# HybridRobotics/ilqr-iterative-tasks

Hardware: AMD Instinct MI355X
Metric: batched iLQR iterations/s (n=6,m=2,N=20) (higher is better)
Workload: dtype f64

## Files before the change

ilqr_iterative_tasks_amd/csrc/i2lqr_abi.hip:

```cpp
#include <hip/hip_runtime.h>

#include <atomic>
#include <cmath>
#include <cstdarg>
#include <cstdio>
#include <cstdlib>
#include <cstring>
#include <mutex>
#include <new>
#include <unordered_set>

#include "../../include/i2lqr.h"
#include "i2lqr_devcfg.hpp"
#include "i2lqr_geometry.hpp"
#include "i2lqr_group.h"
#include "i2lqr_handle.hpp"
#include "i2lqr_host.hpp"
#include "i2lqr_kernels.h"
#include "i2lqr_lane12.h"
#include "i2lqr_rccl.hpp"
#include "i2lqr_select.hpp"
#include "i2lqr_wave_opt.h"

#include "i2lqr_lane_launch.hpp"
// ... 491 lines not shown
  if (!h->lane_models) return refuse_layout(what);
  if (h->cfg.system_id == I2LQR_SYS_QUAD12)
    return fail(I2LQR_ERR_UNSUPPORTED, "%s with \"lane_models\" is built for the bicycles' "
                "one-problem-per-lane kernel, not for quad12's row-block kernel "
                "(k_lane_iterate_rows): use the problem-major layout", what);
  return I2LQR_OK;
}

int i2lqr_set_option(i2lqr_handle* h, const char* name, int64_t value) {
  if (!h || !name) return fail(I2LQR_ERR_INVALID, "null handle or option name");
  if (value < -1 || value > 0x7fffffff) return fail(I2LQR_ERR_INVALID, "option value out of range");
  const int v = (int)value;
  LaneTune& lane = h->lane;
  ColumnTune& col = h->col;
  if (!strcmp(name, "defer_states")) lane.opt_defer = v < 0 ? -1 : (v != 0);
  else if (!strcmp(name, "reroll_nominal")) lane.opt_reroll = v < 0 ? -1 : (v != 0);
  else if (!strcmp(name, "lds_gain_steps")) lane.opt_lds_steps = v;
  else if (!strcmp(name, "merge_inputs")) lane.opt_merge = v < 0 ? -1 : (v != 0);
  else if (!strcmp(name, "checkpoint_states")) lane.opt_ckpt = v < 0 ? -1 : (v != 0);
  else if (!strcmp(name, "stagger")) lane.opt_stagger = v;
  else if (!strcmp(name, "per_step_jacobians")) col.opt_fstep = v < 0 ? -1 : (v != 0);
  else if (!strcmp(name, "wave_tail")) lane.wave_tail = v < 0 ? -1 : (v > 65536 ? 65536 : v);
  else if (!strcmp(name, "first_chunk")) lane.opt_first_chunk = v < 1 ? -1 : (v > 1024 ? 1024 : v);
  else if (!strcmp(name, "helper_wavefront")) lane.opt_pair = v < 0 ? -1 : (v != 0);
  else if (!strcmp(name, "state_buffers")) lane.opt_two_x = v < 0 ? -1 : (v != 0);
  else if (!strcmp(name, "chunk_step")) lane.opt_chunk_step = v < 1 ? -1 : (v > 1024 ? 1024 : v);
  else if (!strcmp(name, "fused_compaction")) lane.opt_fuse = v < 0 ? -1 : (v != 0);
  else if (!strcmp(name, "final_round")) lane.opt_final_round = v < 0 ? -1 : (v > 20 ? 20 : v);
  else if (!strcmp(name, "speculate")) col.opt_spec = v < 0 ? -1 : (v != 0);
  else if (!strcmp(name, "group_workspace")) col.opt_group_ws = v < 0 ? -1 : (v != 0);
  else if (!strcmp(name, "group_overlap")) col.opt_group_overlap = v < 0 ? -1 : (v != 0);
  else if (!strcmp(name, "group_fixed_horizon")) col.opt_group_fixed = v < 0 ? -1 : (v != 0);
  else if (!strcmp(name, "group_chains")) col.opt_group_chains = v < 0 ? -1 : (v != 0);
  else if (!strcmp(name, "debug_self_test")) {
#ifdef I2LQR_DEBUG
    unsigned long long* w = i2lqr::debug_trap_word();
    double* buf = nullptr;
    HIP_TRY(hipMalloc((void**)&buf, 8 * sizeof(double)));
    hipLaunchKernelGGL(k_debug_self_test, dim3(1), dim3(64), 0, (hipStream_t)0, buf, w);
    const int rc = debug_check(I2LQR_OK, nullptr);
    (void)hipFree(buf);
    return rc;
#else
    return fail(I2LQR_ERR_UNSUPPORTED, "\"debug_self_test\" exists in the index-checked debug build "
                "only (make -C ilqr_iterative_tasks_amd/csrc debug)");
#endif
  }
  else if (!strcmp(name, "line_search")) {
    if (v != -1 && v != 0 && v != 1 && v != 2 && v != 4 && v != 8)
      return fail(I2LQR_ERR_INVALID, "\"line_search\" is 2, 4 or 8 step sizes, or -1 / 0 / 1 (off)");
    if (v > 1 && !problem_major(h)) return refuse_layout(wave_phrase(WAVE_LS));
    h->model.ls = v > 1 ? v : 0;
  }
  else if (!strcmp(name, "obstacles")) {
    if (v > I2LQR_MAX_OBSTACLES)
      return fail(I2LQR_ERR_INVALID, "\"obstacles\" is 2 ... %d records per problem, or -1 / 0 / 1 "
                  "(off: one record)", I2LQR_MAX_OBSTACLES);
    if (v > 1)
      if (int rc = refuse_lane_model(h, wave_phrase(WAVE_OBS))) return rc;
    h->model.obs = v > 1 ? v : 0;
  }
  else if (!strcmp(name, "lane_models")) {
    if (v != -1 && v != 0 && v != 1)
      return fail(I2LQR_ERR_INVALID, "\"lane_models\" is 1 (on), or -1 / 0 (off)");
    if (v == 1 && problem_major(h))
      return fail(I2LQR_ERR_UNSUPPORTED, "\"lane_models\" is built for the batch-minor / batch-tiled "
// ... 611 lines not shown
```

ilqr_iterative_tasks_amd/csrc/i2lqr_column_launch.hpp:

```cpp
#pragma once
#include <hip/hip_runtime.h>

#include "i2lqr_column_plan.hpp"
#include "i2lqr_devcfg.hpp"
#include "i2lqr_group.h"
#include "i2lqr_handle.hpp"
#include "i2lqr_host.hpp"
#include "i2lqr_kernels.h"
#include "i2lqr_wave_opt.h"

namespace i2lqr {

inline thread_local i2lqr_handle::Epilogue* t_epi = nullptr;

inline int64_t registered_ws(const i2lqr_handle* h) { return h->ws ? h->ws_bytes : -1; }
inline ColumnChoice column_kernel(const i2lqr_handle* h, int64_t B, bool early_exit) {
  return column_kernel(h->geo, h->fit, h->col, h->model.form(), registered_ws(h), B, early_exit);
}

inline int wave_lds_check(const i2lqr_handle* h, bool chained) {
  const size_t need = wave_lds_need(h->fit, h->model, chained);
  if (need <= h->geo.max_dyn_lds) return I2LQR_OK;
  const WaveForm f = h->model.form(chained);
  const int n_obs = h->model.records();
// ... 6 lines not shown
  return fail(I2LQR_ERR_UNSUPPORTED, "horizon %d with %s needs %zu B of LDS per wavefront (> %zu KiB)",
              h->cfg.N, with, need, h->geo.max_dyn_lds / 1024);
}

template <class T, class Sys> struct Launch {
  static constexpr int n = Sys::n, m = Sys::m, LANES = 64;
  static constexpr bool kBicycle = m == 2 && n + m <= 8;
  using Cfg = DevCfg<T, n, m>;

  static unsigned grid(int64_t B) { return (unsigned)B; }

  static int prepare(i2lqr_handle* h) {
    h->lanes = LANES;
    h->fit.lds_wave = (size_t)Layout<Sys>(h->cfg.N).total * sizeof(T);
    h->fit.lds_wave_fstep = kWaveHasFstep<Sys> ? wave_fstep_lds_bytes<T, Sys>(h->cfg.N) : 0;
    const size_t lds = h->fit.lds_wave;
    if (lds > h->geo.max_dyn_lds)
      return fail(I2LQR_ERR_UNSUPPORTED, "horizon %d needs %zu B of LDS per wavefront (> %zu KiB)",
                  h->cfg.N, lds, h->geo.max_dyn_lds / 1024);
    if (lds > h->geo.default_dyn_lds)
      for (const void* kernel :
           {(const void*)k_iterate<T, Sys, LANES, false>, (const void*)k_iterate<T, Sys, LANES, true>,
            (const void*)k_backward<T, Sys, LANES, false>, (const void*)k_backward<T, Sys, LANES, true>,
            (const void*)k_forward<T, Sys, LANES, false>, (const void*)k_forward<T, Sys, LANES, true>,
            (const void*)k_rollout<T, Sys, LANES, false>, (const void*)k_rollout<T, Sys, LANES, true>})
        HIP_TRY(hipFuncSetAttribute(kernel, hipFuncAttributeMaxDynamicSharedMemorySize, (int)lds));
    return I2LQR_OK;
  }

  static int iterate(i2lqr_handle* h, const SolveIO& io, hipStream_t s) {
    const int64_t B = io.B;
    IterArgs<T> a = iter_args<T>(io);
    a.chains = h->col.opt_group_chains != 0;
#ifdef I2LQR_STAMPS
    a.dbg = (unsigned long long*)h->ws;
#endif
    const ColumnChoice choice = column_kernel(h, B, io.early_exit != 0);
    const ColumnKernel fk = choice.kernel;
    if (t_epi && (fk == K_GROUP || fk == K_GROUP16 || fk == K_GROUP_WS)) {
      a.qfun = t_epi->qfun;
      a.outer_iter = t_epi->outer_iter;
      a.max_relax_iter = t_epi->max_relax_iter;
      a.cost_it = (T*)t_epi->cost_it;
      if (t_epi->best_idx) {
        a.pick_part = (MinPair<T>*)t_epi->part;
        a.pick_ticket = h->ticket + h->ticket_next.fetch_add(1, std::memory_order_relaxed) %
                                        i2lqr_handle::kTickets;
        a.best_idx = t_epi->best_idx;
        a.best_cost = (T*)t_epi->best_cost;
      }
      t_epi->fused = true;
    }
#ifdef I2LQR_STAMPS
    constexpr bool stamps = true;
#else
    constexpr bool stamps = false;
#endif
    switch (fk) {
      case K_INVALID:
        return fail(I2LQR_ERR_UNSUPPORTED, "%s", choice.why);
      case K_SPEC:
      case K_SPEC16:
        if constexpr (kBicycle) {
          const int lanes = fk == K_SPEC16 ? 16 : 8;
          HIP_TRY(group_spec_iterate<T>(h->cfg, a, s, lanes,
                                        spec_wavefronts(h->geo, h->fit, lanes, B, false)));
// ... 106 lines not shown
```

ilqr_iterative_tasks_amd/csrc/i2lqr_column_plan.hpp:

```cpp
#pragma once
#include <cstddef>
#include <cstdint>
#include <cstdio>

#include "../../include/i2lqr.h"
#include "i2lqr_geometry.hpp"
#include "i2lqr_wave_model.hpp"

namespace i2lqr {

struct ColumnTune {
  int opt_fstep = -1;
  int opt_group = -1;
  int opt_spec = -1;
  int opt_group_ws = -1;
  int opt_group_overlap = -1;
  int opt_group_fixed = -1;
  int opt_group_chains = -1;
  int opt_wave_chain = 0;
};

struct ColumnFit {
  enum Plant { OTHER, BICYCLE, SIXTEEN };
  int plant = OTHER;
  bool weights = false;
  bool problem_major = false;
  bool f64 = true;
  int n = 0, N = 0, word = 8;
  bool fixed_horizon = false;
  size_t lds_wave = 0, lds_wave_fstep = 0;
  size_t lds_group8 = 0, lds_group16 = 0;
  size_t lds_group_ws = 0;
  size_t lds_spec8x2 = 0, lds_spec8x3 = 0;
  size_t lds_spec16x2 = 0, lds_spec16x3 = 0;
  size_t lds_quad = 0;
  int64_t ws_group = 0, ws_quad = 0;
};

constexpr int kEightLaneProblems = 8, kSixteenLaneProblems = 4;

constexpr int64_t kAutoGroupBatch = 1024;
constexpr int64_t kAutoSpecBatch = 12288;
constexpr int64_t kGroup16Batch = 4096;
constexpr int64_t kGroupWsBatch = 4096;
constexpr int64_t kGroupWsTop = 8192;
constexpr int64_t kGroupWsTopF32 = 7168;
constexpr int kSpecWideBatch = 512;

inline bool lds_fits(const DeviceGeometry& g, size_t bytes) { return bytes <= g.max_dyn_lds; }
inline bool column_plant_ok(const ColumnFit& f) { return f.plant == ColumnFit::BICYCLE && !f.weights; }
inline bool group_fits(const DeviceGeometry& g, const ColumnFit& f, int lanes) {
// ... 230 lines not shown
```

ilqr_iterative_tasks_amd/csrc/i2lqr_dryrun.hpp:

```cpp
#pragma once
#ifdef I2LQR_DRY_RUN
#include <hip/hip_runtime.h>

#include <cstddef>
#include <cstdint>

#include "i2lqr_wave.hpp"

namespace i2lqr {
namespace dry {

bool on();
void allow(const void* base, size_t bytes);
void reset();
void record(const char* expr, const void* kernel, dim3 grid, dim3 block, size_t lds);
void ptr(const char* field, const void* p);
void val(const char* field, int64_t v);
void end();
int64_t report(char* buf, int64_t n);

template <class A> inline void arg(const A&) {}
inline void arg(int64_t v) { val("int", v); }
inline void arg(int v) { val("int", v); }
template <class P> inline void arg(P* p) { ptr("pointer argument", (const void*)p); }
template <class T> inline void arg(const IterArgs<T>& a) {
  val("IterArgs.B", a.B); val("IterArgs.n_iters", a.n_iters); val("IterArgs.early_exit", a.early_exit);
  ptr("IterArgs.X", a.X); ptr("IterArgs.U", a.U); ptr("IterArgs.x_term", a.x_term);
  ptr("IterArgs.lamb", a.lamb); ptr("IterArgs.obs", a.obs); ptr("IterArgs.cost", a.cost);
  ptr("IterArgs.K", a.K); ptr("IterArgs.k", a.k); ptr("IterArgs.iters", a.iters);
  ptr("IterArgs.status", a.status); ptr("IterArgs.dbg", a.dbg); ptr("IterArgs.count", a.count);
  val("IterArgs.count_max", a.count_max); val("IterArgs.max_total", a.max_total);
  val("IterArgs.set_stride", a.set_stride);
  ptr("IterArgs.orig", a.orig); ptr("IterArgs.out_X", a.out_X);
  ptr("IterArgs.out_U", a.out_U); ptr("IterArgs.out_K", a.out_K);
  ptr("IterArgs.out_k", a.out_k); ptr("IterArgs.out_lamb", a.out_lamb);
  ptr("IterArgs.out_cost", a.out_cost); ptr("IterArgs.out_iters", a.out_iters);
  ptr("IterArgs.out_status", a.out_status);
  val("IterArgs.out_B", a.out_B); val("IterArgs.out_tiled", a.out_tiled);
  ptr("IterArgs.qfun", a.qfun);
  val("IterArgs.outer_iter", a.outer_iter); val("IterArgs.max_relax_iter", a.max_relax_iter);
  ptr("IterArgs.cost_it", a.cost_it); ptr("IterArgs.pick_part", a.pick_part);
  ptr("IterArgs.pick_ticket", a.pick_ticket); ptr("IterArgs.best_idx", a.best_idx);
  ptr("IterArgs.best_cost", a.best_cost); val("IterArgs.chain_len", a.chain_len);
  val("IterArgs.chains", a.chains);
}
#ifdef I2LQR_DRY_RUN_LANE
template <class T> inline void arg(const LaneSet<T>& s) {
  ptr("LaneSet.X", s.X); ptr("LaneSet.U", s.U); ptr("LaneSet.x_term", s.x_term);
  ptr("LaneSet.obs", s.obs); ptr("LaneSet.lamb", s.lamb); ptr("LaneSet.cost", s.cost);
  ptr("LaneSet.K", s.K); ptr("LaneSet.k", s.k); ptr("LaneSet.iters", s.iters);
  ptr("LaneSet.status", s.status); ptr("LaneSet.orig", s.orig); val("LaneSet.B", s.B);
}
template <class T> inline void arg(const LaneArgs<T>& a) {
  val("LaneArgs.B", a.B); val("LaneArgs.n_iters", a.n_iters); val("LaneArgs.early_exit", a.early_exit);
  ptr("LaneArgs.X", a.X); ptr("LaneArgs.U", a.U); ptr("LaneArgs.x_term", a.x_term);
  ptr("LaneArgs.lamb", a.lamb); ptr("LaneArgs.obs", a.obs); ptr("LaneArgs.cost", a.cost);
  ptr("LaneArgs.K", a.K); ptr("LaneArgs.k", a.k); ptr("LaneArgs.iters", a.iters);
  ptr("LaneArgs.status", a.status); ptr("LaneArgs.wsU", a.wsU); ptr("LaneArgs.wsK", a.wsK);
  ptr("LaneArgs.wsk", a.wsk); ptr("LaneArgs.wsX", a.wsX); ptr("LaneArgs.count", a.count);
  val("LaneArgs.resume", a.resume); val("LaneArgs.max_total", a.max_total);
  val("LaneArgs.count_lo", a.count_lo); val("LaneArgs.count_hi", a.count_hi);
  val("LaneArgs.two_max", a.two_max); val("LaneArgs.lds_grow", a.lds_grow);
  ptr("LaneArgs.dbg", a.dbg); val("LaneArgs.defer", a.defer);
  val("LaneArgs.lds_steps", a.lds_steps); val("LaneArgs.reroll", a.reroll);
  val("LaneArgs.merge", a.merge); val("LaneArgs.ckpt", a.ckpt); val("LaneArgs.stagger", a.stagger);
  val("LaneArgs.cp.on", a.cp.on);
  if (a.cp.on) {
    val("LaneArgs.cp.src_is_user", a.cp.src_is_user); val("LaneArgs.cp.user_tiled", a.cp.user_tiled);
    ptr("LaneArgs.cp.orig", a.cp.orig); ptr("LaneArgs.cp.count_out", a.cp.count_out);
    arg(a.cp.dst);
    arg(a.cp.usr);
  }
}
#endif

template <class... A>
inline void launch(const char* expr, const void* kernel, dim3 grid, dim3 block, size_t lds,
// ... 30 lines not shown
```

ilqr_iterative_tasks_amd/csrc/i2lqr_group.h:

```cpp
#pragma once
#include <hip/hip_runtime.h>

#include "../../include/i2lqr.h"
#include "i2lqr_column_plan.hpp"
#include "i2lqr_devcfg.hpp"
#include "i2lqr_wave.hpp"

namespace i2lqr {

inline ColumnFit column_fit_config(const i2lqr_config& cfg) {
  ColumnFit f;
  f.plant = cfg.m == 2 && cfg.n + cfg.m <= 8 ? ColumnFit::BICYCLE
            : cfg.n + cfg.m == 16 ? ColumnFit::SIXTEEN : ColumnFit::OTHER;
  f.weights = has_stage_weights(cfg);
  f.problem_major = cfg.layout == I2LQR_LAYOUT_PROBLEM_MAJOR;
  f.f64 = cfg.dtype == I2LQR_F64;
  f.n = cfg.n;
  f.N = cfg.N;
  f.word = f.f64 ? 8 : 4;
  return f;
}
void column_fit_group(const i2lqr_config& cfg, ColumnFit& fit);
void column_fit_quad(const i2lqr_config& cfg, ColumnFit& fit);

template <class T> hipError_t group_iterate(const i2lqr_config& cfg, const IterArgs<T>& a,
                                            hipStream_t stream, int wavefronts);

template <class T> hipError_t group16_iterate(const i2lqr_config& cfg, const IterArgs<T>& a,
                                              hipStream_t stream, int wavefronts, bool fixed);
#define I2LQR_GROUP_FIXED_HORIZONS(X) X(20)
bool group16_fixed_horizon(int N);
template <class T> hipError_t group16_iterate_fixed(const i2lqr_config& cfg, const IterArgs<T>& a,
                                                    hipStream_t stream, int wavefronts);

template <class T> hipError_t group_iterate_ws(const i2lqr_config& cfg, const IterArgs<T>& a,
                                               void* ws, hipStream_t stream);

template <class T> hipError_t group_spec_iterate(const i2lqr_config& cfg, const IterArgs<T>& a,
                                                 hipStream_t stream, int lanes, int wavefronts);
template <class T> hipError_t group_spec_chain(const i2lqr_config& cfg, const IterArgs<T>& a,
                                               hipStream_t stream);
bool group_spec_tail_supported(const i2lqr_config& cfg);
template <class T> hipError_t group_spec_tail(const i2lqr_config& cfg, const IterArgs<T>& a,
                                              hipStream_t stream);

template <class T> hipError_t quad_iterate(const i2lqr_config& cfg, const IterArgs<T>& a, void* ws,
                                           hipStream_t stream);

}
```

ilqr_iterative_tasks_amd/csrc/i2lqr_group.hip:

```cpp
#include "i2lqr_group.h"

#include "i2lqr_devcfg.hpp"
#include "i2lqr_geometry.hpp"
#include "i2lqr_group.hpp"
#include "i2lqr_dryrun.hpp"
#include "i2lqr_group_launch.hpp"

namespace i2lqr {

namespace {

template <class T, class Sys, int H, int G = kGroup>
hipError_t launch_h(const i2lqr_config& cfg, const IterArgs<T>& a, hipStream_t s) {
  const auto c = make_dev_cfg<T, Sys::n, Sys::m>(cfg);
  const size_t lds = group_lds_bytes<T, Sys, G>(cfg.N);
  if (hipError_t e = raise_lds_limit<k_group_iterate<T, Sys, H, false, G>>(lds); e != hipSuccess)
    return e;
  constexpr int PW = 64 / G;
  const unsigned grid = (unsigned)((a.B + PW - 1) / PW);
  hipLaunchKernelGGL((k_group_iterate<T, Sys, H, false, G>), dim3(grid), dim3(64 * H), lds, s, c, a,
                     (T*)nullptr);
  return hipGetLastError();
}
template <class T, class Sys>
// ... 65 lines not shown
  return spec_tail_lanes(device_geometry(), fit);
}
bool group_spec_tail_supported(const i2lqr_config& cfg) { return group_spec_tail_lanes(cfg) != 0; }

template <class T, class Sys>
hipError_t launch_spec_chain(const i2lqr_config& cfg, const IterArgs<T>& a, hipStream_t s) {
  const auto c = make_dev_cfg<T, Sys::n, Sys::m>(cfg);
  const size_t lds = spec_lds_bytes<T, Sys, 3, 16>(cfg.N);
  if (hipError_t e = raise_lds_limit<k_group_spec<T, Sys, 3, false, 16, true>>(lds); e != hipSuccess)
    return e;
  const unsigned grid = (unsigned)((a.B + 3) / 4);
  hipLaunchKernelGGL((k_group_spec<T, Sys, 3, false, 16, true>), dim3(grid), dim3(64 * 3), lds, s, c, a);
  return hipGetLastError();
}
template <class T>
hipError_t group_spec_chain(const i2lqr_config& cfg, const IterArgs<T>& a, hipStream_t s) {
  return visit_bicycle<T>(cfg, [&](auto, auto sys) {
    return launch_spec_chain<T, decltype(sys)>(cfg, a, s);
  });
}
template <class T>
hipError_t group_spec_iterate(const i2lqr_config& cfg, const IterArgs<T>& a, hipStream_t s, int lanes,
                              int wavefronts) {
  return launch_spec_any<T, false>(cfg, a, s, lanes, wavefronts);
}
template <class T>
hipError_t group_spec_tail(const i2lqr_config& cfg, const IterArgs<T>& a, hipStream_t s) {
  return launch_spec_any<T, true>(cfg, a, s, group_spec_tail_lanes(cfg), 2);
}

template <class T>
hipError_t group16_iterate(const i2lqr_config& cfg, const IterArgs<T>& a, hipStream_t s, int wavefronts,
                           bool fixed) {
  if (fixed) return group16_iterate_fixed<T>(cfg, a, s, wavefronts);
  return visit_bicycle<T>(cfg, [&](auto, auto sys) {
    using Sys = decltype(sys);
    if (wavefronts == 3) return launch_h<T, Sys, 3, 16>(cfg, a, s);
    if (wavefronts == 2) return launch_h<T, Sys, 2, 16>(cfg, a, s);
    return launch_h<T, Sys, 1, 16>(cfg, a, s);
  });
}

template <class T>
hipError_t group_iterate_ws(const i2lqr_config& cfg, const IterArgs<T>& a, void* ws, hipStream_t s) {
  return visit_bicycle<T>(cfg, [&](auto, auto sys) {
    return launch_ws<T, decltype(sys)>(cfg, a, ws, s);
  });
}

template <class T>
hipError_t group_iterate(const i2lqr_config& cfg, const IterArgs<T>& a, hipStream_t s, int wavefronts) {
  return visit_bicycle<T>(cfg, [&](auto, auto sys) {
    using Sys = decltype(sys);
    if (wavefronts == 3) return launch_h<T, Sys, 3>(cfg, a, s);
    return launch_h<T, Sys, 1>(cfg, a, s);
  });
}

#define I2LQR_GROUP_LAUNCHERS(T)                                                                    \
  template hipError_t group_iterate<T>(const i2lqr_config&, const IterArgs<T>&, hipStream_t, int);  \
  template hipError_t group16_iterate<T>(const i2lqr_config&, const IterArgs<T>&, hipStream_t, int, \
                                         bool);                                                    \
  template hipError_t group_iterate_ws<T>(const i2lqr_config&, const IterArgs<T>&, void*,           \
                                          hipStream_t);                                             \
  template hipError_t group_spec_iterate<T>(const i2lqr_config&, const IterArgs<T>&, hipStream_t,   \
                                            int, int);                                              \
  template hipError_t group_spec_chain<T>(const i2lqr_config&, const IterArgs<T>&, hipStream_t);    \
  template hipError_t group_spec_tail<T>(const i2lqr_config&, const IterArgs<T>&, hipStream_t);
I2LQR_GROUP_LAUNCHERS(double)
I2LQR_GROUP_LAUNCHERS(float)

}
```

ilqr_iterative_tasks_amd/csrc/i2lqr_group.hpp:

```cpp
#pragma once
#include <hip/hip_runtime.h>
#include <stdint.h>

#include "i2lqr_systems.hpp"
#include "i2lqr_wave.hpp"

namespace i2lqr {

constexpr int kGroup = 8;
constexpr int kGroupsPerWave = 64 / kGroup;

template <class Sys> struct GroupPattern {
  static constexpr int n = Sys::n, m = Sys::m, W = n + m, NV = Sys::NVAR;
  static constexpr int dt_row(int b) {
    for (int i = 2; i < n; i++)
      if (i != b && Sys::pat(i, b) == 2) return i;
    return -1;
  }
  static constexpr bool column_ok(int b) {
    int extra = 0;
    for (int i = 0; i < n; i++) {
      const int code = Sys::pat(i, b);
      if (i < 2) {
        if (code == 2) return false;
// ... 995 lines not shown
      if (t < N) step(t, ga, gb);
    } else {
      if constexpr (I2LQR_GROUP_UNROLL >= 4) {
        for (; t + 3 < N; t += 4) {
          step(t, ga, ga);
          step(t + 1, ga, ga);
          step(t + 2, ga, ga);
          step(t + 3, ga, ga);
        }
      }
      for (; t + 1 < N; t += 2) {
        step(t, ga, ga);
        step(t + 1, ga, ga);
      }
      if (t < N) step(t, ga, ga);
    }
    Sys::template trig_g<GENERAL>(x, tr, bad);
#pragma unroll
    for (int q = 0; q < NT; q++) S[TRn + N * NT + q] = tr[q];
    const T cost = terminal_cost(x, xT);
    wave_sync();
    return cost;
  }
};

__device__ __forceinline__ int idx_div(int e, int d, float rcp_d) {
  int q = (int)((float)e * rcp_d);
  const int r = e - q * d;
  q += (r >= d) ? 1 : 0;
  q -= (r < 0) ? 1 : 0;
  return q;
}

template <class T, class Sys, int H, bool WS, int G, int NH>
__device__ __forceinline__ void group_iterate_body(const DevCfg<T, Sys::n, Sys::m>& c,
                                                   const IterArgs<T>& a, T* ws) {
  static_assert(!(WS && H > 1), "the workspace form runs without helper wavefronts");
  constexpr int n = Sys::n, m = Sys::m, W = n + m;
#ifdef I2LQR_STAMPS
  constexpr bool OVL = false;
#else
  constexpr bool OVL = G == 16 && H >= 3;
#endif
  using GL = GLayout<Sys, G>;
  extern __shared__ __align__(16) unsigned char gsmem_raw[];
  T* smem = reinterpret_cast<T*>(gsmem_raw);
  const int lane = threadIdx.x & 63, hv = threadIdx.x >> 6;
#ifdef I2LQR_STAMPS
  unsigned long long st_k0, st_k1, st_k2, st_k3;
  asm volatile("s_memtime %0\n\ts_waitcnt lgkmcnt(0)" : "=s"(st_k0)::"memory");
#endif
  const int64_t prob0 = (int64_t)blockIdx.x * GL::PW + lane / G;
  const bool real = prob0 < a.B;
  const int64_t prob = real ? prob0 : a.B - 1;
  GroupWorker<T, Sys, WS, G, NH> w(c, smem, lane);
  const int N = NH > 0 ? NH : c.N, g = w.g;
  const float rN = 1.0f / (float)N, rN1 = 1.0f / (float)(N + 1), rnN = 1.0f / (float)(n * N);
  const GL& L = w.L;
  const auto S = w.S;
  if constexpr (WS) w.Wp = ws + prob0 * (int64_t)L.ws_words();

  if (H == 1 || hv == 0) {
    const T* gX = a.X + prob * (int64_t)(n * (N + 1));
    if (g < n) S[L.XU0 + g] = gX[g * (N + 1)];
    const T* gU = a.U + prob * (int64_t)(m * N);
    for (int e = g; e < m * N; e += G) {
      const int aa = idx_div(e, N, rN), t = e - aa * N;
      S[L.XU0 + t * W + n + aa] = gU[e];
    }
    for (int e = lane; e < n * n; e += 64) smem[L.qt_base() + e] = c.Qt[e];
  }
  T xT[n], ob[6];
#pragma unroll
  for (int i = 0; i < n; i++) xT[i] = a.x_term[prob * n + i];
#pragma unroll
  for (int q = 0; q < 6; q++) ob[q] = a.obs ? a.obs[prob * 6 + q] : T(q == 5 ? -1 : 1);
  T lamb = a.lamb[prob];
  wave_sync();

  int cur = 0;
  const T ob_pa = T(1) / (ob[2] * ob[2]), ob_pb = T(1) / (ob[3] * ob[3]);
  int* const ctl = reinterpret_cast<int*>(smem + L.ctl_base());
  if constexpr (H > 1) {
    if (hv > 0) {
      const int h0 = OVL ? hv - 1 : hv, hs = OVL ? H - 1 : H;
      for (;;) {
        __syncthreads();
        const int flags = ctl[8];
        if (!(flags & 1)) break;
        if (flags & 2) {
          const int pc = ctl[lane / G];
          w.prep(pc ? L.XU1 : L.XU0, pc ? L.TR1 : L.TR0, ob, ob_pa, ob_pb, h0 * G + g, hs * G,
                 a.chains != 0);
        }
        __syncthreads();
      }
      if constexpr (OVL) {
        if (real && a.K) {
          T* const gK = a.K + prob * (int64_t)(m * n * N);
          T* const gk = a.k + prob * (int64_t)(m * N);
          for (int t = h0 * G + g; t < N; t += hs * G) {
            const T* Kt = w.gain(t);
            T kv[m][n + 1];
#pragma unroll
            for (int aa = 0; aa < m; aa++)
#pragma unroll
              for (int j = 0; j <= n; j++) kv[aa][j] = Kt[aa * GL::KW + j];
#pragma unroll
            for (int aa = 0; aa < m; aa++) {
#pragma unroll
// ... 136 lines not shown
      }
      T* gk = a.k + prob * (int64_t)(m * N);
      for (int e = g; e < m * N; e += G) {
        const int aa = idx_div(e, N, rN), t = e - aa * N;
        gk[e] = w.gain(t)[aa * GL::KW + n];
      }
    }
    if (g == 0) {
      a.lamb[prob] = lamb;
      a.cost[prob] = cost_ret;
      if (a.iters) a.iters[prob] = it;
      if (a.status) a.status[prob] = status;
    }
#ifdef I2LQR_STAMPS
    asm volatile("s_waitcnt vmcnt(0)\n\ts_memtime %0\n\ts_waitcnt lgkmcnt(0)" : "=s"(st_k3)::"memory");
    w.st_acc[2] = st_k1 - st_k0;
    w.st_acc[3] = st_k2 - st_k1;
    w.st_acc[4] = st_k3 - st_k2;
    if (a.dbg && g == 0)
      for (int q = 0; q < 8; q++) a.dbg[prob * 8 + q] = w.st_acc[q];
#endif
  }
  if (a.qfun) {
    const bool cand = real && g == 0;
    T ci = T(0);
    if (cand) {
      const int XUo = cur ? L.XU1 : L.XU0;
      double ss = 0.0;
#pragma unroll
      for (int i = 0; i < n; i++) {
        const double d = (double)S[XUo + N * W + i] - (double)xT[i];
        ss += d * d;
      }
      ci = (T)relax_cost_value(ss, a.qfun[prob], N, a.outer_iter, a.max_relax_iter);
      a.cost_it[prob] = ci;
    }
    if (a.pick_part) pick_epilogue(a, cand, prob, ci);
  }
}

template <class T, class Sys, int H = 1, bool WS = false, int G = kGroup>
__global__ __launch_bounds__(64 * H) void k_group_iterate(const DevCfg<T, Sys::n, Sys::m> c,
                                                          const IterArgs<T> a, T* ws = nullptr) {
  group_iterate_body<T, Sys, H, WS, G, 0>(c, a, ws);
}

template <class T, class Sys, int H, int NH>
__global__ __launch_bounds__(64 * H) void k_group_iterate_fixed(const DevCfg<T, Sys::n, Sys::m> c,
                                                                const IterArgs<T> a) {
  static_assert(NH > 0, "a compile-time horizon");
  group_iterate_body<T, Sys, H, false, 16, NH>(c, a, nullptr);
}

template <class Sys, int V, int G = kGroup> struct GSpecLayout {
  static constexpr int n = Sys::n, m = Sys::m, W = n + m, NT = Sys::NTRIG;
  static constexpr int PW = 64 / G;
  using GL = GLayout<Sys, G>;
  int N;
  int traj_words, R, var0, var_words, Kk_in_var, T1c_in_var, total;
  __host__ __device__ explicit GSpecLayout(int N_) : N(N_) {
    const int xu = (W * (N + 1) + 3) & ~3, tr = (NT * (N + 1) + 3) & ~3;
    traj_words = xu + tr;
    int o = (V + 1) * traj_words;
    R = o; o += GL::RW * (N + 1); o = (o + 3) & ~3;
    var0 = o;
    Kk_in_var = 0;
    T1c_in_var = (m * GL::KW * N + 3) & ~3;
    var_words = G == kGroup ? (T1c_in_var + kGroup * 2 * ((W + 1) / 2) + 3) & ~3
                            : (T1c_in_var + m * GL::KW + 3) & ~3;
    o += V * var_words;
    if (((o / 4) & 1) == 0) o += 4;
    total = o;
  }
  __host__ __device__ int xu_off(int b) const { return b * traj_words; }
  __host__ __device__ int tr_off(int b) const { return b * traj_words + ((W * (N + 1) + 3) & ~3); }
  __host__ __device__ int group_words() const { return PW * total + n * n + (V + 1) * PW; }
};

template <class T, class Sys, int V, bool SETIO = false, int G = kGroup, bool CHAIN = false>
__global__ __launch_bounds__(64 * V) void k_group_spec(const DevCfg<T, Sys::n, Sys::m> c,
                                                       const IterArgs<T> a) {
  static_assert(!(CHAIN && SETIO), "chains are problem-major batches");
  constexpr int n = Sys::n, m = Sys::m, W = n + m;
  using GL = GLayout<Sys, G>;
// ... 206 lines not shown
```

ilqr_iterative_tasks_amd/csrc/i2lqr_wave.hpp:

```cpp
#pragma once
#include <hip/hip_runtime.h>
#include <stdint.h>

#include <type_traits>

#include "i2lqr_debug.hpp"
#include "i2lqr_systems.hpp"


namespace i2lqr {

enum : int { FLAG_HAS_Q = 1, FLAG_HAS_R = 2 };

template <class T, int n, int m> struct DevCfg {
  int N, max_iter, flags;
  int fast_barrier;
  T dt, eps, lamb_factor, max_lamb;
  T ctrl_q1, ctrl_q2, obs_q1, obs_q2, safety_margin;
  T u_max[m];
  T ctrl_c[m];
  T xtarget[n];
  T Q[n * n], Qt[n * n], R[m * m];
  T sys_par[8];
  T ctrl_q12, ctrl_q122, obs_q12, obs_q122;
// ... 19 lines not shown
  T* U;
  const T* x_term;
  T* lamb;
  const T* obs;
  T* cost;
  T* K;
  T* k;
  int32_t* iters;
  int32_t* status;
  unsigned long long* dbg;
  const int32_t* count;
  int count_max, max_total;
  int64_t set_stride;
  const int32_t* orig = nullptr;
  T* out_X = nullptr;
  T* out_U = nullptr;
  T* out_K = nullptr;
  T* out_k = nullptr;
  T* out_lamb = nullptr;
  T* out_cost = nullptr;
  int32_t* out_iters = nullptr;
  int32_t* out_status = nullptr;
  int64_t out_B = 0;
  int out_tiled = 0;
  const int32_t* qfun = nullptr;
  int outer_iter = 0, max_relax_iter = 0;
  T* cost_it = nullptr;
  MinPair<T>* pick_part = nullptr;
  unsigned* pick_ticket = nullptr;
  int64_t* best_idx = nullptr;
  T* best_cost = nullptr;
  int chain_len = 1;
  int chains = 1;
};

__device__ __forceinline__ double relax_cost_value(double ss, int32_t qf, int N, int outer_iter,
                                                   int max_relax_iter) {
  const double nrm = sqrt(ss);
  double scale = 1.0;
  for (int q = 0; q < outer_iter; q++) scale *= 10.0;
  double out = INFINITY;
  if (qf == 0x7fffffff) return out;
  for (int i = 1; i <= max_relax_iter; i++) {
    if (nrm <= 80.0 * i / scale) { out = (double)qf + N + 100 * i; break; }
    if (nrm > 80.0 * max_relax_iter / scale) break;
  }
  return out;
}

template <class T>
__device__ __forceinline__ void pick_epilogue(const IterArgs<T>& a, bool cand, int64_t prob, T v) {
  T bv = cand ? v : T(0);
  int64_t bi = (cand && v == v) ? prob : -1;
#pragma unroll
  for (int s = 32; s > 0; s >>= 1) {
    const T ov = __shfl_xor(bv, s);
    const int64_t oi = __shfl_xor(bi, s);
    if (oi >= 0 && better(ov, oi, bv, bi)) { bv = ov; bi = oi; }
  }
  const int lane = threadIdx.x & 63;
  unsigned ticket = 0;
  if (lane == 0) {
    __hip_atomic_store(&a.pick_part[blockIdx.x].v, bv, __ATOMIC_RELAXED, __HIP_MEMORY_SCOPE_AGENT);
    __hip_atomic_store(&a.pick_part[blockIdx.x].i, bi, __ATOMIC_RELAXED, __HIP_MEMORY_SCOPE_AGENT);
    __threadfence();
    ticket = atomicInc(a.pick_ticket, gridDim.x - 1);
  }
  ticket = __builtin_amdgcn_readfirstlane(ticket);
  if (ticket != gridDim.x - 1) return;
  __threadfence();
  bv = T(0);
  bi = -1;
  for (unsigned p = lane; p < gridDim.x; p += 64) {
    const T ov = __hip_atomic_load(&a.pick_part[p].v, __ATOMIC_RELAXED, __HIP_MEMORY_SCOPE_AGENT);
    const int64_t oi = __hip_atomic_load(&a.pick_part[p].i, __ATOMIC_RELAXED, __HIP_MEMORY_SCOPE_AGENT);
    if (oi >= 0 && better(ov, oi, bv, bi)) { bv = ov; bi = oi; }
  }
#pragma unroll
  for (int s = 32; s > 0; s >>= 1) {
    const T ov = __shfl_xor(bv, s);
    const int64_t oi = __shfl_xor(bi, s);
    if (oi >= 0 && better(ov, oi, bv, bi)) { bv = ov; bi = oi; }
  }
  if (lane == 0) {
    *a.best_idx = bi;
    *a.best_cost = bi >= 0 ? bv : (T)INFINITY;
  }
}

#ifdef I2LQR_STAMPS
#define STAMP_DECL unsigned long long st_acc[8] = {0, 0, 0, 0, 0, 0, 0, 0}, st_t0 = 0, st_t1 = 0
#define STAMP_BEGIN()                                                            \
  do {                                                                           \
    __builtin_amdgcn_sched_barrier(0);                                           \
    asm volatile("s_memtime %0\n\ts_waitcnt lgkmcnt(0)" : "=s"(st_t0)::"memory"); \
    __builtin_amdgcn_sched_barrier(0);                                           \
  } while (0)
#define STAMP_END(slot)                                                          \
  do {                                                                           \
    __builtin_amdgcn_sched_barrier(0);                                           \
    asm volatile("s_memtime %0\n\ts_waitcnt lgkmcnt(0)" : "=s"(st_t1)::"memory"); \
    __builtin_amdgcn_sched_barrier(0);                                           \
    st_acc[slot] += st_t1 - st_t0;                                               \
    st_t0 = st_t1;                                                               \
  } while (0)
#else
#define STAMP_DECL
#define STAMP_BEGIN()
#define STAMP_END(slot)
#endif

template <int Begin, int End, class F> __device__ __forceinline__ void static_for_i(F&& f) {
  if constexpr (Begin < End) {
    f(std::integral_constant<int, Begin>{});
    static_for_i<Begin + 1, End>(f);
  }
}

__device__ __forceinline__ void wave_sync() {
  __builtin_amdgcn_fence(__ATOMIC_RELEASE, "wavefront");
  __builtin_amdgcn_wave_barrier();
  __builtin_amdgcn_fence(__ATOMIC_ACQUIRE, "wavefront");
}

template <class T, int L> __device__ __forceinline__ T pick(const T (&a)[L], int i) {
  T v = a[0];
#pragma unroll
  for (int q = 1; q < L; q++) v = (i == q) ? a[q] : v;
  return v;
}

template <class T> __device__ __forceinline__ T clip(T v, T lo, T hi);
template <> __device__ __forceinline__ double clip<double>(double v, double lo, double hi) {
  const double r = __builtin_fmin(__builtin_fmax(v, lo), hi);
  return v != v ? v : r;
}
template <> __device__ __forceinline__ float clip<float>(float v, float lo, float hi) {
  const float r = __builtin_fminf(__builtin_fmaxf(v, lo), hi);
  return v != v ? v : r;
}

template <class Sys> struct Layout {
  static constexpr int n = Sys::n, m = Sys::m, W = n + m, NT = Sys::NTRIG;
  int N;
  int X0, X1, U0, U1, Kk, trg, lu, luu, ob, Va, F, T1, H, g, Qt, Fs, total;
  __host__ __device__ explicit Layout(int N_, bool fstep = false) : N(N_) {
    int o = 0;
    X0 = o; o += n * (N + 1);
    X1 = o; o += n * (N + 1);
    U0 = o; o += m * N;
// ... 750 lines not shown
```

Before: 84.40 million.

## Batch group kernel entry loads and use DPP/readlane pick reduction

Reworks the group kernel prologue so the initial state, controls, terminal cost matrix, target state and qfun index are all loaded into registers before any LDS stores. This lets the global loads be in flight together instead of serialised with the stores. The cross-problem argmin epilogue now reads one representative lane per group with readlane and reduces the final partials with DPP row shifts instead of a full shuffle butterfly. The previous entry path is kept behind a new "group_entry" option and compiled as separate former kernels, which adds code size and register pressure.

```diff
diff --git a/ilqr_iterative_tasks_amd/csrc/i2lqr_abi.hip b/ilqr_iterative_tasks_amd/csrc/i2lqr_abi.hip
--- a/ilqr_iterative_tasks_amd/csrc/i2lqr_abi.hip
+++ b/ilqr_iterative_tasks_amd/csrc/i2lqr_abi.hip
@@ -547,6 +547,7 @@
   else if (!strcmp(name, "group_overlap")) col.opt_group_overlap = v < 0 ? -1 : (v != 0);
   else if (!strcmp(name, "group_fixed_horizon")) col.opt_group_fixed = v < 0 ? -1 : (v != 0);
   else if (!strcmp(name, "group_chains")) col.opt_group_chains = v < 0 ? -1 : (v != 0);
+  else if (!strcmp(name, "group_entry")) col.opt_group_entry = v < 0 ? -1 : (v != 0);
   else if (!strcmp(name, "debug_self_test")) {
 #ifdef I2LQR_DEBUG
     unsigned long long* w = i2lqr::debug_trap_word();
diff --git a/ilqr_iterative_tasks_amd/csrc/i2lqr_column_launch.hpp b/ilqr_iterative_tasks_amd/csrc/i2lqr_column_launch.hpp
--- a/ilqr_iterative_tasks_amd/csrc/i2lqr_column_launch.hpp
+++ b/ilqr_iterative_tasks_amd/csrc/i2lqr_column_launch.hpp
@@ -62,6 +62,7 @@
     const int64_t B = io.B;
     IterArgs<T> a = iter_args<T>(io);
     a.chains = h->col.opt_group_chains != 0;
+    a.entry = h->col.opt_group_entry != 0;
 #ifdef I2LQR_STAMPS
     a.dbg = (unsigned long long*)h->ws;
 #endif
diff --git a/ilqr_iterative_tasks_amd/csrc/i2lqr_column_plan.hpp b/ilqr_iterative_tasks_amd/csrc/i2lqr_column_plan.hpp
--- a/ilqr_iterative_tasks_amd/csrc/i2lqr_column_plan.hpp
+++ b/ilqr_iterative_tasks_amd/csrc/i2lqr_column_plan.hpp
@@ -17,6 +17,7 @@
   int opt_group_overlap = -1;
   int opt_group_fixed = -1;
   int opt_group_chains = -1;
+  int opt_group_entry = -1;
   int opt_wave_chain = 0;
 };
 
diff --git a/ilqr_iterative_tasks_amd/csrc/i2lqr_dryrun.hpp b/ilqr_iterative_tasks_amd/csrc/i2lqr_dryrun.hpp
--- a/ilqr_iterative_tasks_amd/csrc/i2lqr_dryrun.hpp
+++ b/ilqr_iterative_tasks_amd/csrc/i2lqr_dryrun.hpp
@@ -42,7 +42,7 @@
   ptr("IterArgs.cost_it", a.cost_it); ptr("IterArgs.pick_part", a.pick_part);
   ptr("IterArgs.pick_ticket", a.pick_ticket); ptr("IterArgs.best_idx", a.best_idx);
   ptr("IterArgs.best_cost", a.best_cost); val("IterArgs.chain_len", a.chain_len);
-  val("IterArgs.chains", a.chains);
+  val("IterArgs.chains", a.chains); val("IterArgs.entry", a.entry);
 }
 #ifdef I2LQR_DRY_RUN_LANE
 template <class T> inline void arg(const LaneSet<T>& s) {
diff --git a/ilqr_iterative_tasks_amd/csrc/i2lqr_group.h b/ilqr_iterative_tasks_amd/csrc/i2lqr_group.h
--- a/ilqr_iterative_tasks_amd/csrc/i2lqr_group.h
+++ b/ilqr_iterative_tasks_amd/csrc/i2lqr_group.h
@@ -36,6 +36,10 @@
 template <class T> hipError_t group_iterate_ws(const i2lqr_config& cfg, const IterArgs<T>& a,
                                                void* ws, hipStream_t stream);
 
+template <class T> hipError_t group_iterate_former(const i2lqr_config& cfg, const IterArgs<T>& a,
+                                                   hipStream_t stream, int lanes, int wavefronts,
+                                                   bool fixed, void* ws);
+
 template <class T> hipError_t group_spec_iterate(const i2lqr_config& cfg, const IterArgs<T>& a,
                                                  hipStream_t stream, int lanes, int wavefronts);
 template <class T> hipError_t group_spec_chain(const i2lqr_config& cfg, const IterArgs<T>& a,
diff --git a/ilqr_iterative_tasks_amd/csrc/i2lqr_group.hip b/ilqr_iterative_tasks_amd/csrc/i2lqr_group.hip
--- a/ilqr_iterative_tasks_amd/csrc/i2lqr_group.hip
+++ b/ilqr_iterative_tasks_amd/csrc/i2lqr_group.hip
@@ -121,6 +121,7 @@
 template <class T>
 hipError_t group16_iterate(const i2lqr_config& cfg, const IterArgs<T>& a, hipStream_t s, int wavefronts,
                            bool fixed) {
+  if (!a.entry) return group_iterate_former<T>(cfg, a, s, 16, wavefronts, fixed, nullptr);
   if (fixed) return group16_iterate_fixed<T>(cfg, a, s, wavefronts);
   return visit_bicycle<T>(cfg, [&](auto, auto sys) {
     using Sys = decltype(sys);
@@ -132,6 +133,7 @@
 
 template <class T>
 hipError_t group_iterate_ws(const i2lqr_config& cfg, const IterArgs<T>& a, void* ws, hipStream_t s) {
+  if (!a.entry) return group_iterate_former<T>(cfg, a, s, kGroup, 1, false, ws);
   return visit_bicycle<T>(cfg, [&](auto, auto sys) {
     return launch_ws<T, decltype(sys)>(cfg, a, ws, s);
   });
@@ -139,6 +141,7 @@
 
 template <class T>
 hipError_t group_iterate(const i2lqr_config& cfg, const IterArgs<T>& a, hipStream_t s, int wavefronts) {
+  if (!a.entry) return group_iterate_former<T>(cfg, a, s, kGroup, wavefronts, false, nullptr);
   return visit_bicycle<T>(cfg, [&](auto, auto sys) {
     using Sys = decltype(sys);
     if (wavefronts == 3) return launch_h<T, Sys, 3>(cfg, a, s);
diff --git a/ilqr_iterative_tasks_amd/csrc/i2lqr_group.hpp b/ilqr_iterative_tasks_amd/csrc/i2lqr_group.hpp
--- a/ilqr_iterative_tasks_amd/csrc/i2lqr_group.hpp
+++ b/ilqr_iterative_tasks_amd/csrc/i2lqr_group.hpp
@@ -1051,7 +1051,7 @@
   return q;
 }
 
-template <class T, class Sys, int H, bool WS, int G, int NH>
+template <class T, class Sys, int H, bool WS, int G, int NH, bool EA = true>
 __device__ __forceinline__ void group_iterate_body(const DevCfg<T, Sys::n, Sys::m>& c,
                                                    const IterArgs<T>& a, T* ws) {
   static_assert(!(WS && H > 1), "the workspace form runs without helper wavefronts");
@@ -1079,22 +1079,66 @@
   const auto S = w.S;
   if constexpr (WS) w.Wp = ws + prob0 * (int64_t)L.ws_words();
 
-  if (H == 1 || hv == 0) {
-    const T* gX = a.X + prob * (int64_t)(n * (N + 1));
-    if (g < n) S[L.XU0 + g] = gX[g * (N + 1)];
-    const T* gU = a.U + prob * (int64_t)(m * N);
-    for (int e = g; e < m * N; e += G) {
-      const int aa = idx_div(e, N, rN), t = e - aa * N;
-      S[L.XU0 + t * W + n + aa] = gU[e];
-    }
-    for (int e = lane; e < n * n; e += 64) smem[L.qt_base() + e] = c.Qt[e];
-  }
-  T xT[n], ob[6];
-#pragma unroll
-  for (int i = 0; i < n; i++) xT[i] = a.x_term[prob * n + i];
-#pragma unroll
-  for (int q = 0; q < 6; q++) ob[q] = a.obs ? a.obs[prob * 6 + q] : T(q == 5 ? -1 : 1);
-  T lamb = a.lamb[prob];
+  T xT[n], ob[6], lamb;
+  int32_t qf = 0;
+  if constexpr (EA) {
+    if (a.obs) {
+#pragma unroll
+      for (int q = 0; q < 6; q++) ob[q] = a.obs[prob * 6 + q];
+    } else {
+#pragma unroll
+      for (int q = 0; q < 6; q++) ob[q] = T(q == 5 ? -1 : 1);
+    }
+    lamb = a.lamb[prob];
+#pragma unroll
+    for (int i = 0; i < n; i++) xT[i] = T(0);
+    if (H == 1 || hv == 0) {
+      static_assert(n * n <= 64, "one word of Q_terminal per lane");
+      constexpr int UT = NH > 0 ? (m * NH + G - 1) / G : 4;
+      const int mN = m * N;
+      const T* gX = a.X + prob * (int64_t)(n * (N + 1));
+      const T* gU = a.U + prob * (int64_t)mN;
+      T r_u[UT];
+      const T r_x0 = gX[(g < n ? g : n - 1) * (N + 1)];
+#pragma unroll
+      for (int k = 0; k < UT; k++) r_u[k] = gU[g + k * G < mN ? g + k * G : mN - 1];
+      const T r_qt = c.Qt[lane < n * n ? lane : n * n - 1];
+#pragma unroll
+      for (int i = 0; i < n; i++) xT[i] = a.x_term[prob * n + i];
+      if (a.qfun) qf = a.qfun[prob];
+      __builtin_amdgcn_sched_barrier(0);
+      if (g < n) S[L.XU0 + g] = r_x0;
+      if (lane < n * n) smem[L.qt_base() + lane] = r_qt;
+      for (int e0 = g;;) {
+#pragma unroll
+        for (int k = 0; k < UT; k++) {
+          const int e = e0 + k * G, aa = idx_div(e, N, rN), t = e - aa * N;
+          if (e < mN) S[L.XU0 + t * W + n + aa] = r_u[k];
+        }
+        if constexpr (NH > 0) break;
+        e0 += UT * G;
+        if (e0 - g >= mN) break;
+#pragma unroll
+        for (int k = 0; k < UT; k++) r_u[k] = gU[e0 + k * G < mN ? e0 + k * G : mN - 1];
+      }
+    }
+  } else {
+    if (H == 1 || hv == 0) {
+      const T* gX = a.X + prob * (int64_t)(n * (N + 1));
+      if (g < n) S[L.XU0 + g] = gX[g * (N + 1)];
+      const T* gU = a.U + prob * (int64_t)(m * N);
+      for (int e = g; e < m * N; e += G) {
+        const int aa = idx_div(e, N, rN), t = e - aa * N;
+        S[L.XU0 + t * W + n + aa] = gU[e];
+      }
+      for (int e = lane; e < n * n; e += 64) smem[L.qt_base() + e] = c.Qt[e];
+    }
+#pragma unroll
+    for (int i = 0; i < n; i++) xT[i] = a.x_term[prob * n + i];
+#pragma unroll
+    for (int q = 0; q < 6; q++) ob[q] = a.obs ? a.obs[prob * 6 + q] : T(q == 5 ? -1 : 1);
+    lamb = a.lamb[prob];
+  }
   wave_sync();
 
   int cur = 0;
@@ -1297,10 +1341,16 @@
         const double d = (double)S[XUo + N * W + i] - (double)xT[i];
         ss += d * d;
       }
-      ci = (T)relax_cost_value(ss, a.qfun[prob], N, a.outer_iter, a.max_relax_iter);
+      const int32_t qfv = EA ? qf : a.qfun[prob];
+      ci = (T)relax_cost_value(ss, qfv, N, a.outer_iter, a.max_relax_iter);
       a.cost_it[prob] = ci;
     }
-    if (a.pick_part) pick_epilogue(a, cand, prob, ci);
+    if (a.pick_part) {
+      if constexpr (EA)
+        pick_epilogue_direct<T, G>(a, cand, prob, ci);
+      else
+        pick_epilogue_former(a, cand, prob, ci);
+    }
   }
 }
 
@@ -1309,12 +1359,23 @@
                                                           const IterArgs<T> a, T* ws = nullptr) {
   group_iterate_body<T, Sys, H, WS, G, 0>(c, a, ws);
 }
+template <class T, class Sys, int H = 1, bool WS = false, int G = kGroup>
+__global__ __launch_bounds__(64 * H) void k_group_iterate_former(const DevCfg<T, Sys::n, Sys::m> c,
+                                                                 const IterArgs<T> a, T* ws = nullptr) {
+  group_iterate_body<T, Sys, H, WS, G, 0, false>(c, a, ws);
+}
 
 template <class T, class Sys, int H, int NH>
 __global__ __launch_bounds__(64 * H) void k_group_iterate_fixed(const DevCfg<T, Sys::n, Sys::m> c,
                                                                 const IterArgs<T> a) {
   static_assert(NH > 0, "a compile-time horizon");
   group_iterate_body<T, Sys, H, false, 16, NH>(c, a, nullptr);
+}
+template <class T, class Sys, int H, int NH>
+__global__ __launch_bounds__(64 * H) void k_group_iterate_fixed_former(
+    const DevCfg<T, Sys::n, Sys::m> c, const IterArgs<T> a) {
+  static_assert(NH > 0, "a compile-time horizon");
+  group_iterate_body<T, Sys, H, false, 16, NH, false>(c, a, nullptr);
 }
 
 template <class Sys, int V, int G = kGroup> struct GSpecLayout {
diff --git a/ilqr_iterative_tasks_amd/csrc/i2lqr_group_former.hip b/ilqr_iterative_tasks_amd/csrc/i2lqr_group_former.hip
--- /dev/null
+++ b/ilqr_iterative_tasks_amd/csrc/i2lqr_group_former.hip
@@ -0,0 +1,80 @@
+#include "i2lqr_group.h"
+
+#include "i2lqr_devcfg.hpp"
+#include "i2lqr_group.hpp"
+#include "i2lqr_dryrun.hpp"
+#include "i2lqr_group_launch.hpp"
+
+namespace i2lqr {
+
+namespace {
+
+template <class T, class Sys, int H, int G>
+hipError_t former_h(const i2lqr_config& cfg, const IterArgs<T>& a, hipStream_t s) {
+  const auto c = make_dev_cfg<T, Sys::n, Sys::m>(cfg);
+  const size_t lds = group_lds_bytes<T, Sys, G>(cfg.N);
+  if (hipError_t e = raise_lds_limit<k_group_iterate_former<T, Sys, H, false, G>>(lds); e != hipSuccess)
+    return e;
+  constexpr int PW = 64 / G;
+  const unsigned grid = (unsigned)((a.B + PW - 1) / PW);
+  hipLaunchKernelGGL((k_group_iterate_former<T, Sys, H, false, G>), dim3(grid), dim3(64 * H), lds, s, c,
+                     a, (T*)nullptr);
+  return hipGetLastError();
+}
+template <class T, class Sys>
+hipError_t former_ws(const i2lqr_config& cfg, const IterArgs<T>& a, void* ws, hipStream_t s) {
+  const auto c = make_dev_cfg<T, Sys::n, Sys::m>(cfg);
+  const size_t lds = (size_t)GLayout<Sys>(cfg.N, true).wave_words() * sizeof(T);
+  if (hipError_t e = raise_lds_limit<k_group_iterate_former<T, Sys, 1, true>>(lds); e != hipSuccess)
+    return e;
+  const unsigned grid = (unsigned)((a.B + kGroupsPerWave - 1) / kGroupsPerWave);
+  hipLaunchKernelGGL((k_group_iterate_former<T, Sys, 1, true>), dim3(grid), dim3(64), lds, s, c, a,
+                     (T*)ws);
+  return hipGetLastError();
+}
+template <class T, class Sys, int H, int NH>
+hipError_t former_fixed_h(const i2lqr_config& cfg, const IterArgs<T>& a, hipStream_t s) {
+  const auto c = make_dev_cfg<T, Sys::n, Sys::m>(cfg);
+  const size_t lds = group_lds_bytes<T, Sys, 16>(cfg.N);
+  if (hipError_t e = raise_lds_limit<k_group_iterate_fixed_former<T, Sys, H, NH>>(lds); e != hipSuccess)
+    return e;
+  const unsigned grid = (unsigned)((a.B + 3) / 4);
+  hipLaunchKernelGGL((k_group_iterate_fixed_former<T, Sys, H, NH>), dim3(grid), dim3(64 * H), lds, s, c,
+                     a);
+  return hipGetLastError();
+}
+template <class T, class Sys, int H>
+hipError_t former_16(const i2lqr_config& cfg, const IterArgs<T>& a, hipStream_t s, bool fixed) {
+  if (fixed) {
+#define I2LQR_X(NH) if (cfg.N == NH) return former_fixed_h<T, Sys, H, NH>(cfg, a, s);
+    I2LQR_GROUP_FIXED_HORIZONS(I2LQR_X)
+#undef I2LQR_X
+    return hipErrorInvalidValue;
+  }
+  return former_h<T, Sys, H, 16>(cfg, a, s);
+}
+
+}
+
+template <class T>
+hipError_t group_iterate_former(const i2lqr_config& cfg, const IterArgs<T>& a, hipStream_t s, int lanes,
+                                int wavefronts, bool fixed, void* ws) {
+  return visit_bicycle<T>(cfg, [&](auto, auto sys) -> hipError_t {
+    using Sys = decltype(sys);
+    if (ws) return former_ws<T, Sys>(cfg, a, ws, s);
+    if (lanes == 16) {
+      if (wavefronts == 3) return former_16<T, Sys, 3>(cfg, a, s, fixed);
+      if (wavefronts == 2) return former_16<T, Sys, 2>(cfg, a, s, fixed);
+      return former_16<T, Sys, 1>(cfg, a, s, fixed);
+    }
+    if (wavefronts == 3) return former_h<T, Sys, 3, kGroup>(cfg, a, s);
+    return former_h<T, Sys, 1, kGroup>(cfg, a, s);
+  });
+}
+
+template hipError_t group_iterate_former<double>(const i2lqr_config&, const IterArgs<double>&,
+                                                 hipStream_t, int, int, bool, void*);
+template hipError_t group_iterate_former<float>(const i2lqr_config&, const IterArgs<float>&,
+                                                hipStream_t, int, int, bool, void*);
+
+}
diff --git a/ilqr_iterative_tasks_amd/csrc/i2lqr_wave.hpp b/ilqr_iterative_tasks_amd/csrc/i2lqr_wave.hpp
--- a/ilqr_iterative_tasks_amd/csrc/i2lqr_wave.hpp
+++ b/ilqr_iterative_tasks_amd/csrc/i2lqr_wave.hpp
@@ -75,6 +75,7 @@
   T* best_cost = nullptr;
   int chain_len = 1;
   int chains = 1;
+  int entry = 1;
 };
 
 __device__ __forceinline__ double relax_cost_value(double ss, int32_t qf, int N, int outer_iter,
@@ -92,7 +93,7 @@
 }
 
 template <class T>
-__device__ __forceinline__ void pick_epilogue(const IterArgs<T>& a, bool cand, int64_t prob, T v) {
+__device__ __forceinline__ void pick_epilogue_former(const IterArgs<T>& a, bool cand, int64_t prob, T v) {
   T bv = cand ? v : T(0);
   int64_t bi = (cand && v == v) ? prob : -1;
 #pragma unroll
@@ -128,6 +129,89 @@
   if (lane == 0) {
     *a.best_idx = bi;
     *a.best_cost = bi >= 0 ? bv : (T)INFINITY;
+  }
+}
+
+template <int Begin, int End, class F> __device__ __forceinline__ void static_for_i(F&& f) {
+  if constexpr (Begin < End) {
+    f(std::integral_constant<int, Begin>{});
+    static_for_i<Begin + 1, End>(f);
+  }
+}
+
+template <class V, class F> __device__ __forceinline__ V map_words(V x, F f) {
+  static_assert(sizeof(V) % 4 == 0, "whole 32-bit words");
+  int w[sizeof(V) / 4];
+  __builtin_memcpy(w, &x, sizeof(V));
+#pragma unroll
+  for (unsigned k = 0; k < sizeof(V) / 4; k++) w[k] = f(w[k]);
+  __builtin_memcpy(&x, w, sizeof(V));
+  return x;
+}
+template <int L, class V> __device__ __forceinline__ V read_lane(V x) {
+  return map_words(x, [](int w) __attribute__((always_inline)) { return __builtin_amdgcn_readlane(w, L); });
+}
+template <int S, class V> __device__ __forceinline__ V row_shr(V x) {
+  return map_words(x, [](int w) __attribute__((always_inline)) {
+    return __builtin_amdgcn_update_dpp(w, w, 0x110 + S, 0xf, 0xf, false);
+  });
+}
+template <class T>
+__device__ __forceinline__ void take_better(T ov, int64_t oi, T& bv, int64_t& bi) {
+  const bool take = oi >= 0 && better(ov, oi, bv, bi);
+  bv = take ? ov : bv;
+  bi = take ? oi : bi;
+}
+
+template <class T, int G>
+__device__ __forceinline__ void pick_epilogue_direct(const IterArgs<T>& a, bool cand, int64_t prob, T v) {
+  constexpr int PW = 64 / G;
+  const T cv = cand ? v : T(0);
+  const int64_t ci = (cand && v == v) ? prob : -1;
+  T bv = read_lane<0>(cv);
+  int64_t bi = read_lane<0>(ci);
+  static_for_i<1, PW>([&](auto q) __attribute__((always_inline)) {
+    take_better(read_lane<q.value * G>(cv), read_lane<q.value * G>(ci), bv, bi);
+  });
+  const unsigned nwg = (unsigned)((a.B + PW - 1) / PW);
+  const unsigned lane = threadIdx.x & 63;
+  unsigned ticket = 0;
+  if (lane == 0) {
+    __hip_atomic_store(&a.pick_part[blockIdx.x].v, bv, __ATOMIC_RELAXED, __HIP_MEMORY_SCOPE_AGENT);
+    __hip_atomic_store(&a.pick_part[blockIdx.x].i, bi, __ATOMIC_RELAXED, __HIP_MEMORY_SCOPE_AGENT);
+    __threadfence();
+    ticket = atomicInc(a.pick_ticket, nwg - 1);
+  }
+  ticket = __builtin_amdgcn_readfirstlane(ticket);
+  if (ticket != nwg - 1) return;
+  __threadfence();
+  bv = T(0);
+  bi = -1;
+  for (unsigned base = 0; base < nwg; base += 4 * 64) {
+    T ov[4];
+    int64_t oi[4];
+#pragma unroll
+    for (int k = 0; k < 4; k++) {
+      const unsigned p = base + 64 * k + lane, pc = p < nwg ? p : nwg - 1;
+      ov[k] = __hip_atomic_load(&a.pick_part[pc].v, __ATOMIC_RELAXED, __HIP_MEMORY_SCOPE_AGENT);
+      oi[k] = __hip_atomic_load(&a.pick_part[pc].i, __ATOMIC_RELAXED, __HIP_MEMORY_SCOPE_AGENT);
+      oi[k] = p < nwg ? oi[k] : -1;
+    }
+#pragma unroll
+    for (int k = 0; k < 4; k++) take_better(ov[k], oi[k], bv, bi);
+  }
+  take_better(row_shr<1>(bv), row_shr<1>(bi), bv, bi);
+  take_better(row_shr<2>(bv), row_shr<2>(bi), bv, bi);
+  take_better(row_shr<4>(bv), row_shr<4>(bi), bv, bi);
+  take_better(row_shr<8>(bv), row_shr<8>(bi), bv, bi);
+  T fv = read_lane<15>(bv);
+  int64_t fi = read_lane<15>(bi);
+  take_better(read_lane<31>(bv), read_lane<31>(bi), fv, fi);
+  take_better(read_lane<47>(bv), read_lane<47>(bi), fv, fi);
+  take_better(read_lane<63>(bv), read_lane<63>(bi), fv, fi);
+  if (lane == 0) {
+    *a.best_idx = fi;
+    *a.best_cost = fi >= 0 ? fv : (T)INFINITY;
   }
 }
 
@@ -152,13 +236,6 @@
 #define STAMP_BEGIN()
 #define STAMP_END(slot)
 #endif
-
-template <int Begin, int End, class F> __device__ __forceinline__ void static_for_i(F&& f) {
-  if constexpr (Begin < End) {
-    f(std::integral_constant<int, Begin>{});
-    static_for_i<Begin + 1, End>(f);
-  }
-}
 
 __device__ __forceinline__ void wave_sync() {
   __builtin_amdgcn_fence(__ATOMIC_RELEASE, "wavefront");
```

Result: no change. 83.91 million (-0.6%).
